# LouisRouss/DiffuLab

Hardware: AMD Instinct MI355X
Metric: train images/sec/node (DiT-S/2 flow-matching, 256x256 latents) (higher is better)
Workload: dtype bf16

## Files before the change

diffulab_amd/_block.py:

```python

from __future__ import annotations

import ctypes
import re
from functools import lru_cache

from ._lib import HEADER_PATH


@lru_cache(maxsize=1)
def slots() -> dict[str, int]:
    text = re.sub(r"/\*.*?\*/", " ", open(HEADER_PATH).read(), flags=re.S)
    body = text[text.index("DL_BLK_X_IN") : text.index("DL_BLK_NPTR")]
    names = re.findall(r"DL_BLK_([A-Z0-9_]+)", "DL_BLK_" + body.split("DL_BLK_", 1)[1])
    out: dict[str, int] = {}
    for n in names:
        if n not in out:
            out[n] = len(out)
    return out


class DitBlock(ctypes.Structure):
    _fields_ = [("p", ctypes.c_void_p * 96)] + [(n, ctypes.c_int64) for n in
                ("B", "N", "D", "H", "F", "ld_mod", "ld_dmod", "ldw_d", "ldw_f", "ldwt_d", "ldwt_f2", "ldwt_3d", "rot")] + [
                    ("eps", ctypes.c_float), ("next_eps", ctypes.c_float), ("row_gemms", ctypes.c_int32), ("tn_slab_floats", ctypes.c_int64), ("max_workgroups", ctypes.c_int32)]

    def set(self, **ptrs) -> "DitBlock":
        idx = slots()
        for k, v in ptrs.items():
            addr = None if v is None else (v if isinstance(v, int) else v.data_ptr())
            self.p[idx[k.upper()]] = addr
        return self
```

diffulab_amd/csrc/block.hip:

```cpp
#include <stdlib.h>

#include "common.h"

static thread_local hipEvent_t g_blk_event = nullptr;
static int fork_to_side(hipStream_t main, hipStream_t side) {
  if (main == side) return 0;
  if (!g_blk_event && hipEventCreateWithFlags(&g_blk_event, hipEventDisableTiming) != hipSuccess) return -1;
  if (hipEventRecord(g_blk_event, main) != hipSuccess) return -1;
  return hipStreamWaitEvent(side, g_blk_event, 0) == hipSuccess ? 0 : -1;
}

extern "C" int dl_stream_wait_stream(dl_stream_t waiter, dl_stream_t waited) {
  if (fork_to_side((hipStream_t)waited, (hipStream_t)waiter) != 0) {
    dl_set_error("dl_stream_wait_stream: %s", hipGetErrorString(hipGetLastError()));
    return DL_ERR_LAUNCH;
  }
  return DL_OK;
}
extern "C" int dl_memset_zero(void* p, int64_t bytes, dl_stream_t stream) {
  DL_CHECK_ARG(p && bytes >= 0, "dl_memset_zero: bad args");
  if (bytes && hipMemsetAsync(p, 0, (size_t)bytes, (hipStream_t)stream) != hipSuccess) {
    dl_set_error("dl_memset_zero: %s", hipGetErrorString(hipGetLastError()));
    return DL_ERR_LAUNCH;
  }
// ... 124 lines not shown
  } else {
    if (v_in_place)
      RUN(dl_attn_bwd_sv(P(Q), P(K), (const char*)P(QKV) + 2 * D * 2, N * 3 * D, dh, 3 * D, P(A), P(DA), (const float*)P(LSE), P(DQ), P(DK),
                         (char*)P(DQKV) + 2 * D * 2, N * 3 * D, dh, 3 * D, B, H, N, dh, sm, main));
    else
      RUN(dl_attn_bwd(P(Q), P(K), P(V), P(A), P(DA), (const float*)P(LSE), P(DQ), P(DK), P(DV), B, H, N, dh, sm, main));
    RUN(dl_qk_norm_rope_bwd(P(DQ), P(DK), v_in_place ? nullptr : P(DV), P(QKV), (const float*)P(QN_SCALE), (const float*)P(KN_SCALE),
                            (const float*)P(ROPE_COS), (const float*)P(ROPE_SIN), (const float*)P(RRMS), P(DQKV), (float*)P(G_QK_SCALE), B, N,
                            H, dh, b->rot, main));
  }
  RUN(wgrad(P(DQKV), 3 * D, P(XM1), D, P(G_QKV), 3 * D, D));
  if (grouped) {
    if (fork_to_side(main, side)) return DL_ERR_LAUNCH;
    RUN(dl_gemm_tn_group(wg, nwg, M, (float*)P(TN_SLAB), b->tn_slab_floats, side_wgs, side));
  }
  if (!rows)
    RUN(dl_gemm_nt(P(DQKV), 3 * D, P(WT_QKV), b->ldwt_3d, P(DXM), D, M, D, 3 * D, nullptr, DL_ACT_NONE, DL_BF16, nullptr, nullptr, 0,
                   nullptr, 0, 1, main));
  if (P(DFEAT)) RUN(dl_add_bf16(P(DX_MID), P(DFEAT), P(DX_MID), M * D, main));
  if (rows) {
    RUN(dl_ln_modulate_gemm_bwd(P(DQKV), 3 * D, P(WT_QKV), b->ldwt_3d, M, 3 * D, P(X_IN), (const float*)P(LN1_W), (const float*)P(LN1_B),
                                P(SCALE1), b->ld_mod, N, (const float*)P(MEAN1), (const float*)P(RSTD1), P(DX_MID), P(DX_OUT),
                                (float*)P(DSCALE1), (float*)P(DSHIFT1), b->ld_dmod, (float*)P(DWB1), P(PREV_T2), P(PREV_GATE2), b->ld_mod,
                                P(PREV_DT2), (float*)P(PREV_DGATE2), D, main));
  } else {
    RUN(dl_ln_modulate_bwd(P(DXM), P(X_IN), (const float*)P(LN1_W), (const float*)P(LN1_B), P(SCALE1), b->ld_mod, N,
                           (const float*)P(MEAN1), (const float*)P(RSTD1), P(DX_MID), P(DX_OUT), (float*)P(DSCALE1), (float*)P(DSHIFT1),
                           b->ld_dmod, (float*)P(DWB1), P(PREV_T2), P(PREV_GATE2), b->ld_mod, P(PREV_DT2), (float*)P(PREV_DGATE2), M, D,
                           main));
  }
  if (fold_here) RUN(fold(P(DWB1), P(G_LN1)));
  return DL_OK;
}
```

diffulab_amd/engine.py:

```python

from __future__ import annotations

import functools
import math
from dataclasses import dataclass, field

import torch
from torch import Tensor

from . import ops, tuning


_PARAM_EPOCH = 0


def bump_param_epoch() -> None:
    global _PARAM_EPOCH
    _PARAM_EPOCH += 1


def _must(ok: bool) -> None:
    if not ok:
        raise RuntimeError("a HIP kernel declined a shape the engine had selected it for")

# ... 976 lines not shown

        serial = tuning.on("DL_WGRAD_SERIAL")
        sw = SideWork(self, grouped_wgs=256, serial=serial, strict=True)
        main, side = sw.main, sw.side

        early_mod = self.reducer is not None and type(self) is DiTEngine and tuning.on("DL_DP_EARLY_MOD")
        self._early_mod_done = early_mod
        w_mod = self.layout.entries[self.mod_name][0]
        b_mod = self.layout.entries[self.layout.mod_b0][0]

        def early_mod_rows(r0: int, r1: int) -> None:
            ops.cast2d_f32_to_bf16(w["dmod32"][:B, r0:r1], w["dmod"][:B, r0:r1])
            ops.gemm_tn(w["dmod"][:, r0:r1], w["se"], self.grads[w_mod + r0 * E : w_mod + r1 * E].view(r1 - r0, E))
            ops.colsum(w["dmod"][:, r0:r1], self.grads[b_mod + r0 : b_mod + r1], B, r1 - r0)

        def block_done(i: int) -> None:
            if self.reducer is None:
                return
            if early_mod:
                sw.run(lambda: early_mod_rows(i * 6 * D, (i + 1) * 6 * D))
            ev_side = side.record_event()
            self.reducer.ready(*self.layer_ranges[i], extra_events=(ev_side,))
            if early_mod:
                self.reducer.ready(w_mod + i * 6 * D * E, w_mod + (i + 1) * 6 * D * E, flush=i < 3)

        native = self._native_blocks() and not serial
        inline_wgrad = tuning.on("DL_WGRAD_INLINE")
        defer_fold = fused and self.reducer is None
        for i in reversed(range(L)):
            dres = dfeats.get(i - 1)
            if native:
                blk = self._block_args(i, True)
                blk.set(dfeat=dres)
                ops.dit_block_bwd(blk, main.cuda_stream, main.cuda_stream if inline_wgrad else side.cuda_stream, sw.side_wgs)
            elif fused:
                dx = self._block_bwd_row_gemms(i, dx, dres, s, sw, not defer_fold)
            else:
                prev = (w["layers"][i - 1]["t2"], (i - 1) * 6 * D + 5 * D, w["wg"][i - 1]["dt2"]) if i > 0 else None
                m = Modulation(mod, dmod, i * 6 * D, D, N, part=(w["dwb"][2 * i], w["dwb"][2 * i + 1]), groups=B)
                dx = self._dit_block_bwd(w["layers"][i], w["wg"][i], f"layers.{i}.", xs[i], dx, prev, dres, s, m, N, cos, sin, sw,
                                         kb=w.get("kb"), dao=w.get("dao"))
            block_done(i)
        join_last = self.reducer is None and tuning.on("DL_JOIN_LAST")
        if not join_last:
            sw.join()
        if defer_fold:
            ent = self.layout.entries
            stride = ent[self.prefixes[1] + "norm_1.weight"][0] - ent[self.prefixes[0] + "norm_1.weight"][0] if L > 1 else 0
            for j, nm in enumerate(("norm_1.weight", "norm_2.weight")):
                ops.reduce_rows_batched_f32(w["dwb"][j], 2 * B * 2 * D, self.G(self.prefixes[0] + nm), stride, L, B, 2 * D)

        self._cond_bwd(dx)
        if join_last:
            sw.join()
        return self._input_grad(dx) if need_dx else None

    _input_only = False

    def _input_grad(self, dx: Tensor) -> Tensor:
        B, H, W = self.geo[0], self.geo[1], self.geo[2]
        dimg = torch.empty(B, self.d.input_channels, H, W, device=self.dev, dtype=torch.float32)
        return ops.patch_embed_dgrad(dx, self.P(self._conv_name), dimg, self.d.patch_size)

    def _qk_scale_sink(self, qk: str) -> Tensor:
        ent = self.layout.entries
        (q0, qs), (k0, ks) = ent[qk + ".query_norm.scale"], ent[qk + ".key_norm.scale"]
        n = k0 - q0 + math.prod(ks)
# ... 85 lines not shown
        else:
            w["scr_last"].zero_()
            ops.gemm_tn(w["dO"], w["xf"], w["scr_last"], M=_rup(Fo, 8), N=D, scratch=scratch)
            ops.reduce_rows_f32(w["scr_last"], gl, 1, Fo * D)
        ops.colsum(w["dO"], self.G("last_layer.linear.bias"), M, Fo, scratch=scratch)
        if dxm is not None:
            ops.gemm_nt(w["dO"], self.sh["last_layer.linear.weight|t"], dxm, M=M, N=D, K=self._ko)

    def _dfeat_rows(self, dfeats: dict[int, Tensor] | None) -> dict[int, Tensor]:
        return {k: g.reshape(-1, self.d.inner_dim).to(torch.bfloat16).contiguous() for k, g in (dfeats or {}).items()}

    def _patch_wgrad(self, dx: Tensor, name: str, scratch: Tensor | None) -> None:
        d, w = self.d, self.ws
        D, Fi = d.inner_dim, d.input_channels * d.patch_size**2
        gc = self.G(name).view(D, Fi)
        if Fi % 8 == 0:
            ops.gemm_tn(dx, w["tokP"], gc, M=D, N=Fi, scratch=scratch)
        else:
            w["scr_conv"].zero_()
            ops.gemm_tn(dx, w["tokP"], w["scr_conv"], M=D, N=_rup(Fi, 8), scratch=scratch)
            gc.add_(w["scr_conv"][:, :Fi])

    def _end_block(self, sw: "SideWork", bi: int) -> None:
        sw.flush()
        if self.reducer is not None:
            self.reducer.ready(*self.layer_ranges[bi], extra_events=(sw.side.record_event(),))

    def _cond_bwd(self, dx: Tensor, extra_demb: Tensor | None = None) -> None:
        d, w, sh = self.d, self.ws, self.sh
        B, _, _, _, _, _, M, _, _ = self.geo
        D, E = d.inner_dim, d.embedding_dim
        dmod = w["dmod32"]
        det = w.get("det_scr")
        self._patch_wgrad(dx, self._conv_name, det)

        R = self.layout.mod_rows
        g_modw = self.grads[self.layout.entries[self.mod_name][0] :][: R * E].view(R, E)
        g_modb = self.grads[self.layout.entries[self.layout.mod_b0][0] :][:R]
        L6 = len(self.prefixes) * 6 * D if getattr(self, "_early_mod_done", False) else 0
        if L6:
            ops.cast2d_f32_to_bf16(dmod[:B, L6:], w["dmod"][:B, L6:])
            dmod = w["dmod"]
            ops.gemm_tn(dmod[:, L6:], w["se"], g_modw[L6:], scratch=det)
            ops.colsum(dmod[:, L6:], g_modb[L6:], B, R - L6, scratch=det)
        else:
            ops.cast_f32_to_bf16(dmod[:B], w["dmod"][:B])
            dmod = w["dmod"]
            ops.gemm_tn(dmod, w["se"], g_modw, scratch=det)
            ops.colsum(dmod, g_modb, B, R, scratch=det)
        ops.gemm_nt(dmod, sh["@mod|t"], w["dse"], M=B, N=E, K=R, scratch=det)
        table = d.n_classes is not None
        if self._pooled_dim:
            ops.cond_combine_dense_bwd(w["dse"][:B], w["emb"][:B], w["demb"][:B], w["demb16"][:B])
            self._pooled_bwd(B, det)
        else:
            ops.cond_combine_bwd(w["dse"][:B], w["emb"][:B], self._yeff if table else None, w["demb"][:B], w["demb16"][:B],
                                 self.G("label_embed.embedding.weight") if table else None)
        if extra_demb is not None:
            w["demb"][:B].add_(extra_demb[:B])
            ops.cast_f32_to_bf16(w["demb"][:B], w["demb16"][:B])
        ops.colsum(w["demb"], self.G("time_embed.2.bias"), B, E, scratch=det)
        ops.gemm_tn(w["demb16"], w["h1"], self.G("time_embed.2.weight"), scratch=det)
        ops.gemm_nt(w["demb16"], sh["time_embed.2.weight|t"], w["dh1"], M=B, N=E, K=E)
        ops.silu_bwd(w["dh1"][:B], w["pre1"][:B], w["dpre1"][:B])
        ops.gemm_tn(w["dpre1"], w["temb"], self.G("time_embed.0.weight"), scratch=det)
        ops.colsum(w["dpre1"], self.G("time_embed.0.bias"), B, E, scratch=det)
        if self.reducer is not None:
            if L6:
                w_mod = self.layout.entries[self.mod_name][0]
                self.reducer.ready(0, w_mod)
                self.reducer.ready(w_mod + L6 * E, self.layer_ranges[0][0])
            else:
                self.reducer.ready(0, self.layer_ranges[0][0])
            self.reducer.finish()


class _StrictWgradGroups(ops.WgradGroups):

    def _issue(self, key: int) -> None:
        probs = self.pending.pop(key, [])
        if probs:
            self.launch(lambda: _must(ops.gemm_tn_group(probs, self.slab, max_wgs=self.max_wgs)))


class _NoSideWork:

    def wgrad(self, dy: Tensor, x: Tensor, name: str) -> None:
        pass

    def fold(self, partial: Tensor | None, name: str, groups: int) -> None:
        pass

    def flush(self) -> None:
        pass

    def join(self) -> None:
        pass


# ... 35 lines not shown
```

diffulab_amd/ops.py:

```python

from __future__ import annotations

import ctypes
import os

import torch
from torch import Tensor

from ._lib import lib
from . import tuning

BF16, F32 = 0, 1
ACT_NONE, ACT_SILU, ACT_GELU = 0, 1, 2
LOSS_FLOW, LOSS_EPS = 0, 1
MEAN_TYPES = {"epsilon": 0, "xstart": 1, "xprev": 2, "v": 3}
VAR_MODES = {"learned": 0, "learned_range": 1}
VAR_FIXED = -1
PATCH_CPP, PATCH_PPC = 0, 1


_raw_stream = getattr(torch._C, "_cuda_getCurrentRawStream", None)


def _s() -> int:
# ... 535 lines not shown
    gemm_nt(dt, w2t, dh)
    swiglu_bwd(dh, u, du)


def mlp_dswiglu_recompute(x: Tensor, wp: Tensor, dt: Tensor, w2t: Tensor, du: Tensor) -> bool:
    M, F = x.shape[0], w2t.shape[0]
    return _maybe("dl_mlp_dswiglu_recompute", _p(x), x.stride(0), _p(wp), wp.stride(0), _p(dt), dt.stride(0), _p(w2t), w2t.stride(0),
                  _p(du), du.stride(0), M, F, x.shape[1], dt.shape[1], _s())


def _padded_rows(t: Tensor) -> Tensor:
    base = t._base
    if base is not None and base.dim() == t.dim() and base.shape[1:] == t.shape[1:] and base.data_ptr() == t.data_ptr() \
            and base.shape[0] == (t.shape[0] + 63) // 64 * 64 and base.stride() == t.stride():
        return base
    return t


def gemm_tn(a: Tensor, b: Tensor, out: Tensor, *, M: int | None = None, N: int | None = None, max_wgs: int = 0,
            scratch: Tensor | None = None) -> Tensor:
    M = a.shape[1] if M is None else M
    N = b.shape[1] if N is None else N
    if a.shape[0] % 64:
        a, b = _padded_rows(a), _padded_rows(b)
        assert a.shape[0] == b.shape[0], "gemm_tn operands with a ragged row count must be zero-padded row buffers"
    if scratch is not None:
        _call("dl_gemm_tn_det", _p(a), a.stride(0), _p(b), b.stride(0), _p(out), out.stride(0), M, N, a.shape[0], _p(scratch),
              scratch.numel(), _s())
        return out
    _call("dl_gemm_tn_ex", _p(a), a.stride(0), _p(b), b.stride(0), _p(out), out.stride(0), M, N, a.shape[0], int(max_wgs), _s())
    return out


class _WGrad(ctypes.Structure):

    _fields_ = [("dy", ctypes.c_void_p), ("ld_dy", ctypes.c_int64), ("x", ctypes.c_void_p), ("ld_x", ctypes.c_int64),
                ("g", ctypes.c_void_p), ("m_out", ctypes.c_int64), ("n_in", ctypes.c_int64)]


def gemm_tn_group(probs: list[tuple[Tensor, Tensor, Tensor]], slab: Tensor, max_wgs: int = 0) -> bool:
    arr = (_WGrad * len(probs))()
    if probs[0][0].shape[0] % 64:
        probs = [(_padded_rows(dy), _padded_rows(x), g) for dy, x, g in probs]
    R = probs[0][0].shape[0]
    for q, (dy, x, g) in zip(arr, probs):
        assert dy.shape[0] == R and x.shape[0] == R and g.is_contiguous()
        q.dy, q.ld_dy, q.x, q.ld_x, q.g, q.m_out, q.n_in = _p(dy), dy.stride(0), _p(x), x.stride(0), _p(g), g.shape[0], g.shape[1]
    global _LIB
    if _LIB is None:
        _LIB = lib()
    fn = _LIB._fns["dl_gemm_tn_group"][0]
    rc = fn(ctypes.addressof(arr), len(probs), R, _p(slab), slab.numel(), int(max_wgs), _s())
    if rc == -3:
        return False
    if rc != 0:
        raise RuntimeError(f"dl_gemm_tn_group failed ({rc}): {_LIB.cdll.dl_last_error().decode()}")
    return True


_SCRATCH: dict = {}


def shared_scratch(device, floats: int) -> Tensor:
    key = (torch.device(device).type, torch.device(device).index)
    buf = _SCRATCH.get(key)
    if buf is None or buf.numel() < floats:
# ... 158 lines not shown
def attn_fwd(q, k, v, out, lse, B, H, N, dh, scale):
    _call("dl_attn_fwd", _p(q), _p(k), _p(v), _p(out), _p(lse), B, H, N, dh, float(scale), _s())


def attn_bwd(q, k, v, out, dout, lse, dq, dk, dv, B, H, N, dh, scale):
    _call("dl_attn_bwd", _p(q), _p(k), _p(v), _p(out), _p(dout), _p(lse), _p(dq), _p(dk), _p(dv), B, H, N, dh,
          float(scale), _s())


ATTN_MAX_TOKENS = 32768
_INT32_ELEMS = 2 ** 31


def check_row_extent(rows: int, width: int, what: str) -> None:
    if rows * width >= _INT32_ELEMS:
        raise NotImplementedError(f"{what}: {rows} token rows x {width} columns = {rows * width} elements exceed the 2^31 elements the "
                                  "bf16 regime's kernels index; use a smaller batch")


def attn_needs_padding(N: int) -> bool:
    return N % 64 != 0 or (N > 256 and N % 256 != 0)


def v_in_place(N: int) -> bool:
    return N <= 256 and N % 64 == 0 and tuning.on("DL_ATTN_V_IN_PLACE")


def dit_block_fwd(blk, train: bool) -> None:
    _call("dl_dit_block_fwd", ctypes.addressof(blk), int(train), _s())


def dit_block_bwd(blk, main_stream: int, side_stream: int, side_wgs: int) -> None:
    _call("dl_dit_block_bwd", ctypes.addressof(blk), main_stream, side_stream, int(side_wgs))


def attn_fwd_qkv(q, k, qkv, out, lse, B, H, N, dh, scale):
    D = H * dh
    _call("dl_attn_fwd_sv", _p(q), _p(k), qkv.data_ptr() + 2 * D * 2, N * 3 * D, dh, 3 * D, _p(out), _p(lse), B, H, N, dh,
          float(scale), _s())


def gemm_nt_ssq(a, w_sh, out, ssq) -> bool:
    return _maybe("dl_gemm_nt_ssq", _p(a), a.stride(0), _p(w_sh), w_sh.stride(0), _p(out), out.stride(0), a.shape[0], w_sh.shape[0],
                  a.shape[1], _p(ssq), ssq.shape[1], _s())


def attn_fwd_qkn(qkv, ssq, scale_q, scale_k, cos, sin, q, k, rrms, out, lse, B, H, N, dh, rot, scale, eps=1e-6):
    _call("dl_attn_fwd_qkn", _p(qkv), _p(ssq), _p(scale_q), _p(scale_k), _p(cos), _p(sin), float(eps), rot, _p(q), _p(k), _p(rrms), _p(out),
          _p(lse), B, H, N, dh, float(scale), _s())


def attn_bwd_qkv(q, k, qkv, out, dout, lse, dq, dk, dqkv, B, H, N, dh, scale):
    D = H * dh
    _call("dl_attn_bwd_sv", _p(q), _p(k), qkv.data_ptr() + 2 * D * 2, N * 3 * D, dh, 3 * D, _p(out), _p(dout), _p(lse), _p(dq),
          _p(dk), dqkv.data_ptr() + 2 * D * 2, N * 3 * D, dh, 3 * D, B, H, N, dh, float(scale), _s())


def attn_bwd_tok(q, k, qkv, out, dout, lse, dqkv, B, H, N, dh, scale):
    _call("dl_attn_bwd_tok", _p(q), _p(k), _p(qkv), _p(out), _p(dout), _p(lse), _p(dqkv), B, H, N, dh, float(scale), _s())


def qk_inplace_ok(ws: dict, B: int, tokens: int) -> bool:
    return ws.get("qk_part") is not None and v_in_place(tokens) and B * tokens >= 32768


def qk_norm_rope_bwd_inplace(qkv, scale_q, scale_k, cos, sin, rrms, dqkv, dscale, partials, B, N, H, dh, rot, pos=None) -> bool:
# ... 756 lines not shown
```

include/diffulab_hip.h:

```cpp
#ifndef DIFFULAB_HIP_H
#define DIFFULAB_HIP_H

#include <stdint.h>

#ifdef __cplusplus
extern "C" {
#endif

#define DL_API __attribute__((visibility("default")))

typedef void* dl_stream_t;

enum { DL_OK = 0, DL_ERR_INVALID = -1, DL_ERR_LAUNCH = -2, DL_ERR_UNSUPPORTED = -3 };
enum { DL_BF16 = 0, DL_F32 = 1 };
enum { DL_ACT_NONE = 0, DL_ACT_SILU = 1, DL_ACT_GELU = 2 };
enum { DL_LOSS_FLOW = 0, DL_LOSS_EPS = 1 };
enum { DL_MEAN_EPSILON = 0, DL_MEAN_XSTART = 1, DL_MEAN_XPREV = 2, DL_MEAN_V = 3 };
enum { DL_VAR_LEARNED = 0, DL_VAR_LEARNED_RANGE = 1 };
enum { DL_VAR_FIXED = -1 };
enum { DL_PATCH_CPP = 0, DL_PATCH_PPC = 1 };

DL_API int dl_version(void);
DL_API const char* dl_last_error(void);
DL_API int dl_device_info(int device, int* cu_count, int* lds_bytes_per_cu, int64_t* hbm_bytes, char* arch,
// ... 131 lines not shown
  void* C;
  int64_t ldc;
  int64_t M, N, K;
  const float* bias;
  const void* resid;
  int64_t ldr;
} dl_nt_problem_t;
DL_API int dl_gemm_nt_pair(const dl_nt_problem_t* problems, int n, dl_stream_t stream);
DL_API int dl_gemm_nt_swiglu(const void* X, int64_t ldx, const void* Wp, int64_t ldw, void* U, int64_t ldu, void* H,
                             int64_t ldh, int64_t M, int64_t F, int64_t K, dl_stream_t stream);
DL_API int dl_mlp_dswiglu_recompute(const void* X, int64_t ldx, const void* Wp, int64_t ldwp, const void* dT, int64_t ldt,
                                    const void* W2t, int64_t ldw2, void* dU, int64_t lddu, int64_t M, int64_t F, int64_t K1,
                                    int64_t K2, dl_stream_t stream);
DL_API int dl_gemm_tn(const void* A, int64_t lda, const void* B, int64_t ldb, float* C, int64_t ldc, int64_t M,
                      int64_t N, int64_t R, dl_stream_t stream);
DL_API int dl_gemm_tn_ex(const void* A, int64_t lda, const void* B, int64_t ldb, float* C, int64_t ldc, int64_t M,
                         int64_t N, int64_t R, int max_workgroups, dl_stream_t stream);
typedef struct dl_wgrad_t {
  const void* dy;
  int64_t ld_dy;
  const void* x;
  int64_t ld_x;
  float* g;
  int64_t m_out, n_in;
} dl_wgrad_t;
DL_API int dl_gemm_tn_group(const dl_wgrad_t* probs, int n_probs, int64_t R, float* slab, int64_t slab_floats, int max_workgroups,
                            dl_stream_t stream);
DL_API int dl_gemm_tn_det(const void* A, int64_t lda, const void* B, int64_t ldb, float* C, int64_t ldc, int64_t M, int64_t N,
                          int64_t R, float* scratch, int64_t scratch_floats, dl_stream_t stream);
DL_API int dl_gemm_nt_f32_det(const void* A, int64_t lda, const void* B, int64_t ldb, float* C, int64_t ldc, int64_t M, int64_t N,
                              int64_t K, float* scratch, int64_t scratch_floats, dl_stream_t stream);
DL_API int dl_colsum_det(const void* x, int dtype, int64_t ld, float* out, int64_t R, int64_t C, float* scratch,
                         int64_t scratch_floats, dl_stream_t stream);

DL_API int dl_ln_modulate_fwd(const void* x, const float* w, const float* b, const void* scale, const void* shift,
                              int64_t ld_mod, int64_t rows_per_mod, float eps, void* out, float* mean,
                              float* rstd, const void* t, const void* gate, int64_t ld_gate, void* x_out, int64_t M,
                              int64_t D, dl_stream_t stream);
DL_API int dl_ln_modulate_bwd(const void* dout, const void* x, const float* w, const float* b, const void* scale,
                              int64_t ld_mod, int64_t rows_per_mod, const float* mean, const float* rstd,
                              const void* dres, void* dx, float* dscale, float* dshift, int64_t ld_dmod,
                              float* dwb_partial, const void* gate_t, const void* gate, int64_t ld_gate, void* dt,
                              float* dgate, int64_t M, int64_t D, dl_stream_t stream);
DL_API int dl_ln_modulate_bwd_tok(const void* dout, const void* x, const float* w, const float* b, const void* scale,
                                  int64_t ld_mod, const float* mean, const float* rstd, const void* dres, void* dx, void* dscale,
                                  void* dshift, int64_t ld_dmod, float* dwb_partial, int64_t n_part, const void* gate_t,
                                  const void* gate, int64_t ld_gate, void* dt, void* dgate, int64_t M, int64_t D,
                                  dl_stream_t stream);
DL_API int dl_ln_modulate_gemm_fwd(const void* A, int64_t lda, const void* W, int64_t ldw, int64_t M, int64_t K, const void* resid,
                                   const void* gate, int64_t ld_gate, const float* ln_w, const float* ln_b, const void* scale,
                                   const void* shift, int64_t ld_mod, int64_t rows_per_mod, float eps, void* t_out, void* x_out,
                                   void* xm_out, float* mean, float* rstd, int64_t D, dl_stream_t stream);
DL_API int dl_ln_modulate_gemm_bwd(const void* A, int64_t lda, const void* Wt, int64_t ldw, int64_t M, int64_t K, const void* x,
                                   const float* ln_w, const float* ln_b, const void* scale, int64_t ld_mod, int64_t rows_per_mod,
                                   const float* mean, const float* rstd, const void* dres, void* dx, float* dscale, float* dshift,
                                   int64_t ld_dmod, float* dwb_partial, const void* gate_t, const void* gate, int64_t ld_gate,
                                   void* dt, float* dgate, int64_t D, dl_stream_t stream);
DL_API int dl_gemm_nt_qk_norm_rope(const void* A, int64_t lda, const void* Wqkv, int64_t ldw, int64_t B, int64_t N, int64_t H,
                                   int64_t dh, int64_t rot, float eps, const float* scale_q, const float* scale_k, const float* cos,
                                   const float* sin, void* qkv, void* q, void* k, float* rrms, int64_t n_dst, int64_t n_off,
                                   dl_stream_t stream);
DL_API int dl_ddt_cond_fwd(const void* enc, int64_t ld, const float* temb, int64_t ld_t, int64_t B, int64_t N, int64_t D, void* out,
                           dl_stream_t stream);
DL_API int dl_ddt_cond_bwd(const void* dsz, const void* enc, int64_t ld, const float* temb, int64_t ld_t, int64_t B, int64_t N,
                           int64_t D, void* denc, float* dtemb, dl_stream_t stream);
DL_API int dl_gate_bwd(const void* dout, const void* t, const void* gate, int64_t ld_mod, int64_t rows_per_mod,
// ... 324 lines not shown
  DL_BLK_DT2,
  DL_BLK_DX_IN,
  DL_BLK_DX_MID,
  DL_BLK_DX_OUT,
  DL_BLK_DH, DL_BLK_DU, DL_BLK_DXM, DL_BLK_DT1, DL_BLK_DA, DL_BLK_DQ, DL_BLK_DK, DL_BLK_DV, DL_BLK_DQKV, DL_BLK_DFEAT ,
  DL_BLK_DSCALE1, DL_BLK_DSHIFT1, DL_BLK_DGATE1, DL_BLK_DSCALE2, DL_BLK_DSHIFT2,
  DL_BLK_DWB1, DL_BLK_DWB2,
  DL_BLK_PREV_T2, DL_BLK_PREV_GATE2, DL_BLK_PREV_DT2, DL_BLK_PREV_DGATE2,
  DL_BLK_G_QKV, DL_BLK_G_PROJ, DL_BLK_G_UP, DL_BLK_G_DOWN, DL_BLK_G_LN1, DL_BLK_G_LN2, DL_BLK_G_QK_SCALE,
  DL_BLK_NEXT_LN_W, DL_BLK_NEXT_LN_B, DL_BLK_NEXT_SCALE, DL_BLK_NEXT_SHIFT,
  DL_BLK_NEXT_X,
  DL_BLK_NEXT_XM, DL_BLK_NEXT_MEAN, DL_BLK_NEXT_RSTD,
  DL_BLK_TN_SLAB,
  DL_BLK_QK_PARTIALS,
  DL_BLK_SSQ,
  DL_BLK_NPTR
};
typedef struct dl_dit_block_t {
  void* p[96];
  int64_t B, N, D, H, F;
  int64_t ld_mod, ld_dmod;
  int64_t ldw_d, ldw_f;
  int64_t ldwt_d, ldwt_f2, ldwt_3d;
  int64_t rot;
  float eps;
  float next_eps;
  int32_t row_gemms;
  int64_t tn_slab_floats;
  int32_t max_workgroups;
} dl_dit_block_t;
DL_API int dl_dit_block_fwd(const dl_dit_block_t* blk, int train, dl_stream_t stream);
DL_API int dl_dit_block_bwd(const dl_dit_block_t* blk, dl_stream_t main_stream, dl_stream_t side_stream, int side_workgroups);

#ifdef __cplusplus
}
#endif
#endif
```

Measured before the change: 12400.

## Add native conditioning backward with skinny weight-gradient GEMM kernel

Moves the conditioning-path backward (mod, time-embed and patch-embed weight gradients, combine, silu) into one native C entry point so it is no longer a sequence of Python-dispatched ops. A new skinny TN GEMM kernel handles the small-batch weight gradients and fuses the bias column sums (via an MFMA against ones) and the f32-to-bf16 cast of dmod into the same pass. The last block's backward also stops giving workgroups to the side stream when there is no reducer. The risks are a new hand-written kernel with LDS swizzle and transpose-read correctness concerns, and a fallback path whenever the shape constraints are not met.

```diff
diff --git a/diffulab_amd/_block.py b/diffulab_amd/_block.py
--- a/diffulab_amd/_block.py
+++ b/diffulab_amd/_block.py
@@ -20,6 +20,39 @@
     return out
 
 
+@lru_cache(maxsize=1)
+def _cond_fields() -> list[tuple[str, object]]:
+    text = re.sub(r"/\*.*?\*/", " ", open(HEADER_PATH).read(), flags=re.S)
+    body = re.search(r"typedef struct dl_cond_bwd_t \{(.*?)\} dl_cond_bwd_t;", text, flags=re.S).group(1)
+    fields: list[tuple[str, object]] = []
+    for decl in body.split(";"):
+        decl = " ".join(decl.split())
+        if not decl:
+            continue
+        ctype = ctypes.c_void_p if "*" in decl else ctypes.c_int64
+        assert ctype is ctypes.c_void_p or decl.startswith("int64_t "), decl
+        names = decl.split("*")[-1] if "*" in decl else decl[len("int64_t "):]
+        fields += [(n.strip(), ctype) for n in names.split(",")]
+    return fields
+
+
+def cond_bwd_struct(**members):
+    cls = _cond_struct()
+    c = cls()
+    kinds = dict(_cond_fields())
+    assert set(members) == set(kinds), sorted(set(members) ^ set(kinds))
+    for k, v in members.items():
+        if kinds[k] is ctypes.c_void_p:
+            v = None if v is None else (v if isinstance(v, int) else v.data_ptr())
+        setattr(c, k, v)
+    return c
+
+
+@lru_cache(maxsize=1)
+def _cond_struct():
+    return type("CondBwd", (ctypes.Structure,), {"_fields_": _cond_fields()})
+
+
 class DitBlock(ctypes.Structure):
     _fields_ = [("p", ctypes.c_void_p * 96)] + [(n, ctypes.c_int64) for n in
                 ("B", "N", "D", "H", "F", "ld_mod", "ld_dmod", "ldw_d", "ldw_f", "ldwt_d", "ldwt_f2", "ldwt_3d", "rot")] + [
diff --git a/diffulab_amd/csrc/block.hip b/diffulab_amd/csrc/block.hip
--- a/diffulab_amd/csrc/block.hip
+++ b/diffulab_amd/csrc/block.hip
@@ -180,3 +180,30 @@
   if (fold_here) RUN(fold(P(DWB1), P(G_LN1)));
   return DL_OK;
 }
+
+extern "C" int dl_cond_bwd(const dl_cond_bwd_t* c, dl_stream_t stream) {
+  DL_CHECK_ARG(c && c->dmod32 && c->dmod && c->se && c->g_modw && c->g_modb && c->wt_mod && c->dse && c->emb && c->demb && c->demb16 &&
+                   c->h1 && c->pre1 && c->temb && c->wt_t2 && c->dh1 && c->dpre1 && c->g_t2w && c->g_t2b && c->g_t0w && c->g_t0b && c->det_scr,
+               "dl_cond_bwd: null operand");
+  const int64_t B = c->B, E = c->E, R = c->R, T = c->T, r0 = c->r_begin;
+  DL_CHECK_ARG(B > 0 && E > 0 && T > 0 && r0 >= 0 && r0 < R, "dl_cond_bwd: bad dims");
+  if (B > 256 || E > 384 || T > 384 || E % 8 || T % 8 || R % 8 || r0 % 8) {
+    dl_set_error("dl_cond_bwd: no skinny weight-gradient kernel for B=%lld E=%lld T=%lld R=%lld", (long long)B, (long long)E, (long long)T,
+                 (long long)R);
+    return DL_ERR_UNSUPPORTED;
+  }
+  if (c->dx) {
+    DL_CHECK_ARG(c->tokP && c->g_conv && c->M_tok % 64 == 0 && c->Fi % 8 == 0, "dl_cond_bwd: patch-embedding operands");
+    RUN(dl_gemm_tn_det(c->dx, c->D, c->tokP, c->ld_tokP, c->g_conv, c->Fi, c->D, c->Fi, c->M_tok, c->det_scr, c->det_floats, stream));
+  }
+  RUN(dl_gemm_tn_skinny(c->dmod32, DL_F32, c->ld_dmod32, c->se, E, c->g_modw, E, c->g_modb, c->dmod, c->ld_dmod, r0, R, E, B, 1, stream));
+  RUN(dl_gemm_nt_f32_det(c->dmod, c->ld_dmod, c->wt_mod, c->ldwt_mod, c->dse, E, B, E, R, c->det_scr, c->det_floats, stream));
+  RUN(dl_cond_combine_bwd(c->dse, c->emb, c->idx, c->demb, c->demb16, c->dtable, B, E, stream));
+  RUN(dl_colsum_det(c->demb, DL_F32, E, c->g_t2b, B, E, c->det_scr, c->det_floats, stream));
+  RUN(dl_gemm_tn_skinny(c->demb16, DL_BF16, E, c->h1, E, c->g_t2w, E, nullptr, nullptr, 0, 0, E, E, B, 1, stream));
+  RUN(dl_gemm_nt(c->demb16, E, c->wt_t2, c->ldwt_t2, c->dh1, E, B, E, E, nullptr, DL_ACT_NONE, DL_F32, nullptr, nullptr, 0, nullptr, 0, 1,
+                 stream));
+  RUN(dl_silu_bwd(c->dh1, c->pre1, c->dpre1, B * E, stream));
+  RUN(dl_gemm_tn_skinny(c->dpre1, DL_BF16, E, c->temb, c->ld_temb, c->g_t0w, T, c->g_t0b, nullptr, 0, 0, E, T, B, 1, stream));
+  return DL_OK;
+}
diff --git a/diffulab_amd/csrc/gemm_skinny.hip b/diffulab_amd/csrc/gemm_skinny.hip
--- /dev/null
+++ b/diffulab_amd/csrc/gemm_skinny.hip
@@ -0,0 +1,209 @@
+#include "common.h"
+
+#define SK_BM 64
+#define SK_BK 64
+#define SK_NMAX 384
+#define SK_THREADS 512
+#define SK_TILE 16384
+#define SK_STAGE (4 * SK_TILE)
+#define SK_LDS (2 * SK_STAGE)
+
+typedef __attribute__((address_space(3))) void lds_void_t;
+
+__device__ __forceinline__ s16x4_t sk_tr16(const char* p) {
+  s16x4_t v;
+  asm volatile("ds_read_b64_tr_b16 %0, %1" : "=v"(v) : "v"((unsigned)(uintptr_t)(lds_void_t*)p));
+  return v;
+}
+template <int NB>
+__device__ __forceinline__ void sk_landed(bf16x8_t& a, bf16x8_t (&b)[NB]) {
+  asm volatile("s_waitcnt lgkmcnt(0)" ::: "memory");
+  asm volatile("" : "+v"(a));
+#pragma unroll
+  for (int j = 0; j < NB; ++j) asm volatile("" : "+v"(b[j]));
+}
+
+template <bool A_F32>
+__global__ __launch_bounds__(SK_THREADS) void gemm_tn_skinny_k(const void* __restrict__ A_, int64_t lda,
+                                                                 const bf16_t* __restrict__ X, int64_t ldx, float* __restrict__ G,
+                                                                 int64_t ldg, float* __restrict__ gb, bf16_t* __restrict__ a16,
+                                                                 int64_t lda16, int m_begin, int m_end, int N, int R, int accumulate) {
+  extern __shared__ __attribute__((aligned(16))) char smem[];
+  const int tid = threadIdx.x, lane = tid & 63;
+  const int wave = __builtin_amdgcn_readfirstlane(tid >> 6);
+  const int wr = wave >> 2, wc = wave & 3;
+  const int m0 = m_begin + blockIdx.x * SK_BM;
+  const int nchunks = (R + SK_BK - 1) / SK_BK;
+  const int xtiles = (N + 127) >> 7;
+
+  const int ar = tid >> 3, aq = tid & 7;
+  const int am = m0 + aq * 8;
+  const bool a_col_ok = am < m_end;
+  const int a_dst = ar * 256 + ((aq ^ ((ar & 3) << 2)) << 4);
+  u32x4_t pa;
+  u32x4_t px[6];
+  auto load = [&](int c) {
+    const int r0 = c * SK_BK;
+    pa = u32x4_t{0u, 0u, 0u, 0u};
+    if (a_col_ok && r0 + ar < R) {
+      if (A_F32) {
+        const float* s = (const float*)A_ + (int64_t)(r0 + ar) * lda + am;
+        const f32x4_t lo = *(const f32x4_t*)s, hi = *(const f32x4_t*)(s + 4);
+        pa = u32x4_t{pack2bf(lo[0], lo[1]), pack2bf(lo[2], lo[3]), pack2bf(hi[0], hi[1]), pack2bf(hi[2], hi[3])};
+      } else {
+        pa = *(const u32x4_t*)((const bf16_t*)A_ + (int64_t)(r0 + ar) * lda + am);
+      }
+    }
+#pragma unroll
+    for (int u = 0; u < 6; ++u) {
+      const int s = tid + SK_THREADS * u;
+      const int r = (s >> 4) & 63, n = (u >> 1) * 128 + (s & 15) * 8;
+      px[u] = u32x4_t{0u, 0u, 0u, 0u};
+      if ((u >> 1) < xtiles && n < N && r0 + r < R) px[u] = *(const u32x4_t*)(X + (int64_t)(r0 + r) * ldx + n);
+    }
+  };
+  auto store = [&](int c, int buf) {
+    char* st = smem + buf * SK_STAGE;
+    *(u32x4_t*)(st + a_dst) = pa;
+    if (a16 != nullptr && a_col_ok && c * SK_BK + ar < R) *(u32x4_t*)(a16 + (int64_t)(c * SK_BK + ar) * lda16 + am) = pa;
+#pragma unroll
+    for (int u = 0; u < 6; ++u) {
+      if ((u >> 1) >= xtiles) continue;
+      const int s = tid + SK_THREADS * u;
+      const int r = (s >> 4) & 63, q = s & 15;
+      *(u32x4_t*)(st + (1 + (u >> 1)) * SK_TILE + r * 256 + ((q ^ ((r & 3) << 2)) << 4)) = px[u];
+    }
+  };
+
+  const int li = lane & 15, g = lane >> 4;
+  auto tr_off = [&](int col_base, int kk, int half) -> int {
+    const int r = kk * 16 + (g >> 1) * 8 + half * 4 + (li >> 2);
+    const int col = col_base + (g & 1) * 16 + (li & 3) * 4;
+    const int slot = (col >> 3) ^ ((r & 3) << 2);
+    return r * 256 + slot * 16 + (col & 7) * 2;
+  };
+  auto frag = [&](const char* tile, int col_base, int kk) -> bf16x8_t {
+    union {
+      s16x4_t h[2];
+      bf16x8_t v;
+    } u;
+    u.h[0] = sk_tr16(tile + tr_off(col_base, kk, 0));
+    u.h[1] = sk_tr16(tile + tr_off(col_base, kk, 1));
+    return u.v;
+  };
+
+  const int nb = wc * 96;
+  const bool sums = gb != nullptr && wc == 0;
+  bf16x8_t ones;
+#pragma unroll
+  for (int e = 0; e < 8; ++e) ones[e] = (__bf16)1.0f;
+
+  f32x16_t tot[3], tot_s;
+#pragma unroll
+  for (int r = 0; r < 16; ++r) tot[0][r] = tot[1][r] = tot[2][r] = tot_s[r] = 0.f;
+
+  load(0);
+  store(0, 0);
+  for (int c = 0; c < nchunks; ++c) {
+    if (c + 1 < nchunks) load(c + 1);
+    __syncthreads();
+    const char* st = smem + (c & 1) * SK_STAGE;
+    f32x16_t acc[3], acc_s;
+#pragma unroll
+    for (int r = 0; r < 16; ++r) acc[0][r] = acc[1][r] = acc[2][r] = acc_s[r] = 0.f;
+    if (nb < N) {
+#pragma unroll
+      for (int kk = 0; kk < 4; ++kk) {
+        bf16x8_t af = frag(st, wr * 32, kk), bfg[3];
+#pragma unroll
+        for (int j = 0; j < 3; ++j) {
+          const int n = nb + 32 * j;
+          bfg[j] = (n < N) ? frag(st + (1 + (n >> 7)) * SK_TILE, n & 127, kk) : ones;
+        }
+        sk_landed(af, bfg);
+#pragma unroll
+        for (int j = 0; j < 3; ++j)
+          if (nb + 32 * j < N) acc[j] = __builtin_amdgcn_mfma_f32_32x32x16_bf16(af, bfg[j], acc[j], 0, 0, 0);
+        if (sums) acc_s = __builtin_amdgcn_mfma_f32_32x32x16_bf16(af, ones, acc_s, 0, 0, 0);
+      }
+#pragma unroll
+      for (int j = 0; j < 3; ++j) tot[j] += acc[j];
+      tot_s += acc_s;
+    }
+    if (c + 1 < nchunks) store(c + 1, (c + 1) & 1);
+  }
+
+  if (nb >= N) return;
+  const int mrow = m0 + wr * 32 + 4 * (lane >> 5);
+  if (accumulate) {
+#pragma unroll
+    for (int j = 0; j < 3; ++j) {
+      if (nb + 32 * j >= N) continue;
+      const int n = nb + 32 * j + (lane & 31);
+      const float* gcol = G + (n < N ? n : N - 1);
+      float old[16];
+#pragma unroll
+      for (int r = 0; r < 16; ++r) {
+        const int m = mrow + (r & 3) + 8 * (r >> 2);
+        old[r] = gcol[(int64_t)(m < m_end ? m : m_end - 1) * ldg];
+      }
+#pragma unroll
+      for (int r = 0; r < 16; ++r) tot[j][r] += old[r];
+    }
+    if (sums) {
+      float old[16];
+#pragma unroll
+      for (int r = 0; r < 16; ++r) {
+        const int m = mrow + (r & 3) + 8 * (r >> 2);
+        old[r] = gb[m < m_end ? m : m_end - 1];
+      }
+#pragma unroll
+      for (int r = 0; r < 16; ++r) tot_s[r] += old[r];
+    }
+  }
+#pragma unroll
+  for (int j = 0; j < 3; ++j) {
+    const int n = nb + 32 * j + (lane & 31);
+#pragma unroll
+    for (int r = 0; r < 16; ++r) {
+      const int m = mrow + (r & 3) + 8 * (r >> 2);
+      if (n < N && m < m_end) G[(int64_t)m * ldg + n] = tot[j][r];
+    }
+  }
+  if (sums && (lane & 31) == 0) {
+#pragma unroll
+    for (int r = 0; r < 16; ++r) {
+      const int m = mrow + (r & 3) + 8 * (r >> 2);
+      if (m < m_end) gb[m] = tot_s[r];
+    }
+  }
+}
+
+extern "C" int dl_gemm_tn_skinny(const void* A, int a_dtype, int64_t lda, const void* X, int64_t ldx, float* G, int64_t ldg, float* gb,
+                                 void* a_bf16_out, int64_t ld_a_out, int64_t m_begin, int64_t m_end, int64_t N, int64_t R,
+                                 int accumulate, dl_stream_t stream) {
+  DL_CHECK_ARG(A && X && G && (a_dtype == DL_BF16 || a_dtype == DL_F32), "dl_gemm_tn_skinny: null operand / dtype");
+  DL_CHECK_ARG(R > 0 && R <= 256 && N > 0 && N <= SK_NMAX && N % 8 == 0, "dl_gemm_tn_skinny: R=%lld (1..256), N=%lld (8..384, %% 8)",
+               (long long)R, (long long)N);
+  DL_CHECK_ARG(m_begin >= 0 && m_end > m_begin && m_begin % 8 == 0 && m_end % 8 == 0 && m_end < (1ll << 31),
+               "dl_gemm_tn_skinny: row range [%lld, %lld) must be non-empty with multiples of 8", (long long)m_begin, (long long)m_end);
+  DL_CHECK_ARG(lda % 8 == 0 && ldx % 8 == 0 && lda >= m_end && ldx >= N && ldg >= N, "dl_gemm_tn_skinny: leading dims (lda=%lld ldx=%lld ldg=%lld)",
+               (long long)lda, (long long)ldx, (long long)ldg);
+  DL_CHECK_ARG((((uintptr_t)A | (uintptr_t)X) & 15) == 0, "dl_gemm_tn_skinny: 16-byte alignment");
+  DL_CHECK_ARG(!a_bf16_out || (ld_a_out % 8 == 0 && ld_a_out >= m_end && ((uintptr_t)a_bf16_out & 15) == 0 && a_dtype == DL_F32),
+               "dl_gemm_tn_skinny: the bf16 copy of A needs an f32 A, ld %% 8 and 16-byte alignment");
+  static DevOnce once;
+  (void)dev_cus(once, [] {
+    (void)hipFuncSetAttribute((const void*)gemm_tn_skinny_k<false>, hipFuncAttributeMaxDynamicSharedMemorySize, SK_LDS);
+    (void)hipFuncSetAttribute((const void*)gemm_tn_skinny_k<true>, hipFuncAttributeMaxDynamicSharedMemorySize, SK_LDS);
+  });
+  const int grid = cdiv(m_end - m_begin, SK_BM);
+  if (a_dtype == DL_F32)
+    hipLaunchKernelGGL(gemm_tn_skinny_k<true>, grid, SK_THREADS, SK_LDS, (hipStream_t)stream, A, lda, (const bf16_t*)X, ldx, G, ldg, gb,
+                       (bf16_t*)a_bf16_out, ld_a_out, (int)m_begin, (int)m_end, (int)N, (int)R, accumulate);
+  else
+    hipLaunchKernelGGL(gemm_tn_skinny_k<false>, grid, SK_THREADS, SK_LDS, (hipStream_t)stream, A, lda, (const bf16_t*)X, ldx, G, ldg, gb,
+                       (bf16_t*)nullptr, (int64_t)0, (int)m_begin, (int)m_end, (int)N, (int)R, accumulate);
+  DL_LAUNCH_CHECK();
+  return DL_OK;
+}
diff --git a/diffulab_amd/engine.py b/diffulab_amd/engine.py
--- a/diffulab_amd/engine.py
+++ b/diffulab_amd/engine.py
@@ -1032,7 +1032,8 @@
             if native:
                 blk = self._block_args(i, True)
                 blk.set(dfeat=dres)
-                ops.dit_block_bwd(blk, main.cuda_stream, main.cuda_stream if inline_wgrad else side.cuda_stream, sw.side_wgs)
+                side_wgs = 0 if i == 0 and self.reducer is None else sw.side_wgs
+                ops.dit_block_bwd(blk, main.cuda_stream, main.cuda_stream if inline_wgrad else side.cuda_stream, side_wgs)
             elif fused:
                 dx = self._block_bwd_row_gemms(i, dx, dres, s, sw, not defer_fold)
             else:
@@ -1184,12 +1185,34 @@
         D, E = d.inner_dim, d.embedding_dim
         dmod = w["dmod32"]
         det = w.get("det_scr")
-        self._patch_wgrad(dx, self._conv_name, det)
-
         R = self.layout.mod_rows
         g_modw = self.grads[self.layout.entries[self.mod_name][0] :][: R * E].view(R, E)
         g_modb = self.grads[self.layout.entries[self.layout.mod_b0][0] :][:R]
         L6 = len(self.prefixes) * 6 * D if getattr(self, "_early_mod_done", False) else 0
+        table = d.n_classes is not None
+        T = d.frequency_embedding
+        if (self._native_blocks() and det is not None and not self._pooled_dim and extra_demb is None and R % 8 == 0 and L6 % 8 == 0
+                and ops.gemm_tn_skinny_ok(B, E, E) and ops.gemm_tn_skinny_ok(B, E, T)):
+            from ._block import cond_bwd_struct
+
+            Fi = d.input_channels * d.patch_size**2
+            patch = Fi % 8 == 0 and M % 64 == 0 and dx.shape[0] == M
+            if not patch:
+                self._patch_wgrad(dx, self._conv_name, det)
+            ops.cond_bwd(cond_bwd_struct(
+                B=B, E=E, R=R, T=T, r_begin=L6, dmod32=dmod, ld_dmod32=dmod.stride(0), dmod=w["dmod"], ld_dmod=w["dmod"].stride(0),
+                se=w["se"], g_modw=g_modw, g_modb=g_modb, wt_mod=sh["@mod|t"], ldwt_mod=sh["@mod|t"].stride(0), dse=w["dse"],
+                emb=w["emb"], idx=self._yeff if table else None, demb=w["demb"], demb16=w["demb16"],
+                dtable=self.G("label_embed.embedding.weight") if table else None, h1=w["h1"], pre1=w["pre1"], temb=w["temb"],
+                ld_temb=w["temb"].stride(0), wt_t2=sh["time_embed.2.weight|t"], ldwt_t2=sh["time_embed.2.weight|t"].stride(0),
+                dh1=w["dh1"], dpre1=w["dpre1"], g_t2w=self.G("time_embed.2.weight"), g_t2b=self.G("time_embed.2.bias"),
+                g_t0w=self.G("time_embed.0.weight"), g_t0b=self.G("time_embed.0.bias"), det_scr=det, det_floats=det.numel(),
+                dx=dx if patch else None, tokP=w["tokP"], ld_tokP=w["tokP"].stride(0), g_conv=self.G(self._conv_name), M_tok=M, D=D,
+                Fi=Fi))
+            self._cond_ready(L6)
+            return
+        self._patch_wgrad(dx, self._conv_name, det)
+
         if L6:
             ops.cast2d_f32_to_bf16(dmod[:B, L6:], w["dmod"][:B, L6:])
             dmod = w["dmod"]
@@ -1201,7 +1224,6 @@
             ops.gemm_tn(dmod, w["se"], g_modw, scratch=det)
             ops.colsum(dmod, g_modb, B, R, scratch=det)
         ops.gemm_nt(dmod, sh["@mod|t"], w["dse"], M=B, N=E, K=R, scratch=det)
-        table = d.n_classes is not None
         if self._pooled_dim:
             ops.cond_combine_dense_bwd(w["dse"][:B], w["emb"][:B], w["demb"][:B], w["demb16"][:B])
             self._pooled_bwd(B, det)
@@ -1217,6 +1239,10 @@
         ops.silu_bwd(w["dh1"][:B], w["pre1"][:B], w["dpre1"][:B])
         ops.gemm_tn(w["dpre1"], w["temb"], self.G("time_embed.0.weight"), scratch=det)
         ops.colsum(w["dpre1"], self.G("time_embed.0.bias"), B, E, scratch=det)
+        self._cond_ready(L6)
+
+    def _cond_ready(self, L6: int) -> None:
+        E = self.d.embedding_dim
         if self.reducer is not None:
             if L6:
                 w_mod = self.layout.entries[self.mod_name][0]
diff --git a/diffulab_amd/ops.py b/diffulab_amd/ops.py
--- a/diffulab_amd/ops.py
+++ b/diffulab_amd/ops.py
@@ -591,6 +591,24 @@
     return out
 
 
+SKINNY_MAX_R, SKINNY_MAX_N = 256, 384
+
+
+def gemm_tn_skinny_ok(R: int, M: int, N: int) -> bool:
+    return 0 < R <= SKINNY_MAX_R and 0 < N <= SKINNY_MAX_N and N % 8 == 0 and M % 8 == 0
+
+
+def gemm_tn_skinny(a: Tensor, b: Tensor, out: Tensor, *, R: int | None = None, N: int | None = None, rows: tuple[int, int] | None = None,
+                   bias_out: Tensor | None = None, a_bf16_out: Tensor | None = None, accumulate: bool = True) -> Tensor:
+    R = a.shape[0] if R is None else R
+    N = b.shape[1] if N is None else N
+    m0, m1 = (0, a.shape[1]) if rows is None else rows
+    assert out.dtype == torch.float32 and b.dtype == torch.bfloat16 and a.dtype in (torch.float32, torch.bfloat16)
+    _call("dl_gemm_tn_skinny", _p(a), F32 if a.dtype == torch.float32 else BF16, a.stride(0), _p(b), b.stride(0), _p(out), out.stride(0),
+          _p(bias_out), _p(a_bf16_out), a_bf16_out.stride(0) if a_bf16_out is not None else 0, m0, m1, N, R, int(accumulate), _s())
+    return out
+
+
 class _WGrad(ctypes.Structure):
 
     _fields_ = [("dy", ctypes.c_void_p), ("ld_dy", ctypes.c_int64), ("x", ctypes.c_void_p), ("ld_x", ctypes.c_int64),
@@ -815,6 +833,10 @@
 
 def dit_block_bwd(blk, main_stream: int, side_stream: int, side_wgs: int) -> None:
     _call("dl_dit_block_bwd", ctypes.addressof(blk), main_stream, side_stream, int(side_wgs))
+
+
+def cond_bwd(c) -> None:
+    _call("dl_cond_bwd", ctypes.addressof(keep(c)), _s())
 
 
 def attn_fwd_qkv(q, k, qkv, out, lse, B, H, N, dh, scale):
diff --git a/include/diffulab_hip.h b/include/diffulab_hip.h
--- a/include/diffulab_hip.h
+++ b/include/diffulab_hip.h
@@ -187,6 +187,9 @@
                               int64_t K, float* scratch, int64_t scratch_floats, dl_stream_t stream);
 DL_API int dl_colsum_det(const void* x, int dtype, int64_t ld, float* out, int64_t R, int64_t C, float* scratch,
                          int64_t scratch_floats, dl_stream_t stream);
+DL_API int dl_gemm_tn_skinny(const void* A, int a_dtype, int64_t lda, const void* X, int64_t ldx, float* G, int64_t ldg, float* gb,
+                             void* a_bf16_out, int64_t ld_a_out, int64_t m_begin, int64_t m_end, int64_t N, int64_t R,
+                             int accumulate, dl_stream_t stream);
 
 DL_API int dl_ln_modulate_fwd(const void* x, const float* w, const float* b, const void* scale, const void* shift,
                               int64_t ld_mod, int64_t rows_per_mod, float eps, void* out, float* mean,
@@ -577,6 +580,46 @@
 DL_API int dl_dit_block_fwd(const dl_dit_block_t* blk, int train, dl_stream_t stream);
 DL_API int dl_dit_block_bwd(const dl_dit_block_t* blk, dl_stream_t main_stream, dl_stream_t side_stream, int side_workgroups);
 
+typedef struct dl_cond_bwd_t {
+  int64_t B, E, R, T;
+  int64_t r_begin;
+  const float* dmod32;
+  int64_t ld_dmod32;
+  void* dmod;
+  int64_t ld_dmod;
+  const void* se;
+  float* g_modw;
+  float* g_modb;
+  const void* wt_mod;
+  int64_t ldwt_mod;
+  float* dse;
+  const float* emb;
+  const int64_t* idx;
+  float* demb;
+  void* demb16;
+  float* dtable;
+  const void* h1;
+  const void* pre1;
+  const void* temb;
+  int64_t ld_temb;
+  const void* wt_t2;
+  int64_t ldwt_t2;
+  float* dh1;
+  void* dpre1;
+  float* g_t2w;
+  float* g_t2b;
+  float* g_t0w;
+  float* g_t0b;
+  float* det_scr;
+  int64_t det_floats;
+  const void* dx;
+  const void* tokP;
+  int64_t ld_tokP;
+  float* g_conv;
+  int64_t M_tok, D, Fi;
+} dl_cond_bwd_t;
+DL_API int dl_cond_bwd(const dl_cond_bwd_t* c, dl_stream_t stream);
+
 #ifdef __cplusplus
 }
 #endif
```

Measured after the change: 12440 (median of 6 runs). About the same (+0.4%).
